# jizongFox/Self-paced-Contrastive-Learning

Measured on AMD Instinct MI355X. Metric: pretrain slices/sec/node (UNet+InfoNCE, 224^2, bs=32/GPU), higher is better.
Workload: dtype bf16; 1 GPU; BASELINE.json configs[1]: self-paced pretrain step, UNet base (max_channel=256) encoder to Conv5 + ProjectionHead(256,256,256) + SelfPacedSupConLoss(soft, partition labels, correct_grad) fwd+bwd + RAdam; slices_per_gpu=32, images_per_gpu_step=64, image=1x224x224, global_batch=32, parallelism=dp1, params=1311056, hipgraph=epocher, capture_steps=3

## Files before the change

include/spcl_hip.h:

```cpp
#ifndef SPCL_HIP_H
#define SPCL_HIP_H
#include <stddef.h>
#include <stdint.h>
#ifdef __cplusplus
extern "C" {
#endif

#define SPCL_F32 0
#define SPCL_BF16 1

#define SPCL_OK 0
#define SPCL_EINVAL (-1)
#define SPCL_ELAUNCH (-2)
#define SPCL_EUNSUPPORTED (-3)

#define SPCL_ABI_VERSION 23
int spcl_abi_version(void);
const char* spcl_last_error(void);

size_t spcl_supcon_workspace_bytes(int n, int d);
int spcl_supcon_forward(const float* z1, const float* z2, const float* labels, const float* mask, int n, int d,
                        float temperature, int sp_mode, float gamma, int correct_grad, float* ws, float* out,
                        void* stream);
int spcl_supcon_backward(const float* labels, const float* mask, int n, int d, float temperature, int sp_mode,
                         float gamma, const float* ws_fwd, float* ws_bwd, const float* out_fwd,
                         const float* grad_out, float* dz1, float* dz2, void* stream);
size_t spcl_supcon_bwd_workspace_bytes(int n, int d);
int spcl_supcon_unit_gradient_block(int n, int d, size_t* offset_floats, int* row_pitch);
int spcl_supcon_forward_heads(int K, const float* z1, const float* z2, size_t z_stride, const float* labels, int n,
                              int d, float temperature, int sp_mode, const float* gammas, int correct_grad, float* ws,
                              size_t ws_stride, float* out, void* stream);
int spcl_supcon_rows_supported(int n, int d);
int spcl_supcon_forward_rows(int K, const float* o1, const float* o2, size_t o_stride, const float* labels, int n, int d,
                             float temperature, int sp_mode, const float* gammas, int correct_grad, float* ws,
                             size_t ws_stride, float* out, void* stream);
int spcl_supcon_backward_heads(int K, const float* labels, int n, int d, float temperature, int sp_mode,
                               const float* gammas, const float* ws_fwd, size_t ws_stride, float* ws_bwd,
                               size_t wsb_stride, const float* out_fwd, const float* grad_out, float* dz1, float* dz2,
                               size_t z_stride, void* stream);
int spcl_supcon_materialize(const float* labels, const float* mask, int n, int d, float temperature, int sp_mode,
                            float gamma, const float* ws_fwd, float* sim_logits, float* sim_exp, float* pos_mask,
                            float* neg_mask, float* sp_mask, void* stream);

size_t spcl_supcon_xpos_workspace_bytes(int n, int d);
int spcl_supcon_xpos_forward(const float* z1, const float* z2, const float* labels, const float* mask, int n, int d,
                             float temperature, float* ws, float* out, void* stream);
int spcl_supcon_xpos_backward(const float* z1, const float* z2, int n, int d, float temperature, const float* ws,
                              const float* grad_out, float* dz1, float* dz2, void* stream);

// ... 172 lines not shown
int spcl_bnrelu_backward_bcast(const void* y, const void* dact_nc, int dtype, int N, int H, int W, int C, int CS,
                               const float* mean, const float* invstd, const float* scale, const float* shift, int training,
                               float* ws, float* dgamma, float* dbeta, void* dy, void* stream);

size_t spcl_bnrelu_image_wgrad_workspace_bytes(int N, int H, int W, int CS);
int spcl_bnrelu_backward_image_wgrad(const void* y, const void* dact, const float* image, int dtype, int N, int H,
                                     int W, int C, int CS, const float* mean, const float* invstd, const float* scale,
                                     const float* shift, int training, float* ws, float* dgamma, float* dbeta,
                                     float* dw, void* stream);

int spcl_conv_dgrad_bnstats_supported(int dtype, int N, int H, int W, int CinK, int CoutS);
int spcl_conv3x3_dgrad_bnstats(const void* dy, int dtype, int N, int H, int W, int CinK, int CoutS, const void* w_packed,
                               void* g, const void* y2, const float* scale2, const float* shift2, const float* mean2,
                               float* rows2, void* stream);

int spcl_image_autocorr_rows(int N, int H, int W);
int spcl_image_autocorr(const float* image, int N, int H, int W, float* out, void* stream);
int spcl_conv_dgrad_bnstats_image_supported(int dtype, int N, int H, int W, int CinK, int CoutS);
int spcl_conv3x3_dgrad_bnstats_image(const void* dy, int dtype, int N, int H, int W, int CinK, int CoutS,
                                     const void* w_packed, void* g, const void* y2, const float* scale2,
                                     const float* shift2, const float* mean2, const float* image, float* rows11,
                                     void* stream);
int spcl_conv16_bwd_fused_supported(int dtype, int N, int H, int W, int CinK, int CoutS);
int spcl_conv16_bwd_fused_splits(int N, int H, int W);
int spcl_conv16_bwd_fused(const void* dy, int dtype, int N, int H, int W, const void* w_packed_dgrad, const void* y2,
                          const float* scale2, const float* shift2, const float* mean2, const float* image,
                          float* rows11, float* partial, float* dw_oihw, int Cin, int Cout, float* wg_rows,
                          const float* acorr, int nacorr, float* acorr16, void* stream);
int spcl_conv16_bwd_fused_image_supported(int dtype, int N, int H, int W, int CinK, int CoutS);
int spcl_conv16_bwd_fused_image(const void* dy, int dtype, int N, int H, int W, const void* w_packed_dgrad,
                                const void* w_packed_image, const float* scale2, const float* shift2, const float* mean2,
                                const float* image, float* rows11, float* partial, float* dw_oihw, int Cin, int Cout,
                                float* wg_rows, const float* acorr, int nacorr, float* acorr16, void* stream);
int spcl_bnrelu_backward_wgrows_image3(const float* wg_rows, int nwg, const float* acorr, int nacorr, const float* w_oihw,
                                       int N, int H, int W, int C, int CS, const float* mean, const float* invstd,
                                       const float* scale, int training, float* ws, float* dgamma, float* dbeta,
                                       float* dw, void* stream);
size_t spcl_bnrelu_image3_workspace_bytes(int CS);
int spcl_bnrelu_backward_rows_image3(const float* rows11, int nrows, const float* acorr, int nacorr, const float* w_oihw,
                                     int N, int H, int W, int C, int CS, const float* mean, const float* invstd,
                                     const float* scale, int training, float* ws, float* dgamma, float* dbeta, float* dw,
                                     void* stream);

int spcl_conv_dgrad_poolstats_supported(int dtype, int N, int H, int W, int CinK, int CoutS, int H2, int W2);
int spcl_conv3x3_dgrad_poolstats(const void* dy, int dtype, int N, int H, int W, int CinK, int CoutS, const void* w_packed,
                                 void* g, const void* y2, int H2, int W2, const float* scale2, const float* shift2,
                                 const float* mean2, float* rows2, void* stream);
int spcl_bnrelu_pool_backward_rows(const void* y, const void* dpool, const float* rows, int nrows, int dtype, int N, int H,
                                   int W, int C, int CS, const float* mean, const float* invstd, const float* scale,
                                   const float* shift, int training, float* ws, float* dgamma, float* dbeta, void* dy,
                                   void* stream);
int spcl_bnrelu_backward_rows(const void* y, const void* dact, const float* image, const float* rows, int nrows, int dtype,
                              int N, int H, int W, int C, int CS, const float* mean, const float* invstd,
                              const float* scale, const float* shift, int training, float* ws, float* dgamma,
                              float* dbeta, void* dy, float* dw, void* stream);


int spcl_conv1x1_forward(const void* x, int dtype, size_t npix, int C, int CS, int K, const float* w, const float* b,
                         float* out, void* stream);
size_t spcl_conv1x1_bwd_workspace_bytes(int C, int K);
int spcl_conv1x1_backward(const void* x, const float* dout, int dtype, size_t npix, int C, int CS, int K, const float* w,
                          void* dx, float* dw, float* db, float* ws, void* stream);
int spcl_conv1x1_forward_bn(const void* y, int dtype, size_t npix, int C, int CS, int K, const float* scale,
                            const float* shift, const float* w, const float* b, float* out, void* stream);
int spcl_conv1x1_bwd_rows(size_t npix);
int spcl_conv1x1_backward_bn(const void* y, const float* dout, int dtype, size_t npix, int C, int CS, int K,
// ... 232 lines not shown
```

self-paced-contrastive-learning_amd/functional.py:

```python
from __future__ import annotations

import ctypes
import math
import os
from ctypes import c_double, c_float, c_int

import torch

from . import native as _n

SP_NONE, SP_HARD, SP_SOFT = 0, 1, 2


def take_grad_sink(param, needed: bool = True):
    if not needed or param is None:
        return None
    sink = getattr(param, "_grad_sink", None)
    if sink is None or not getattr(param, "_grad_sink_armed", False):
        return None
    if sink.shape != param.shape or sink.dtype != torch.float32 or not sink.is_contiguous() or sink.device != param.device:
        return None
    param._grad_sink_armed = False
    return sink

# ... 1357 lines not shown
_CONV16_FUSED = os.environ.get("SPCL_CONV16_FUSED", "1") != "0"
_CONV16_WGROWS = os.environ.get("SPCL_CONV16_WGROWS", "1") != "0"


def _conv16_bwd_fused(dy, wp_t, y2, st2, image, dt_code, N, H, W, cin, cout, cs, sink, acorr=None, wp_image=None):
    dev = dy.device
    if y2 is None and wp_image is None:
        raise RuntimeError("conv16 backward: neither the first convolution's output nor its packed weights")
    nsplit = _n.call("spcl_conv16_bwd_fused_splits", N, H, W)
    if acorr is not None:
        rows = torch.empty(11 * cs * nsplit, dtype=torch.float32, device=dev)
        rows.wg, rows.acorr16 = nsplit, torch.empty(16, 64, dtype=torch.float32, device=dev)
    else:
        nt = _n.call("spcl_conv_stat_rows", dt_code, N, H, W, cs, cs)
        rows = torch.empty(nt * 11 * cs, dtype=torch.float32, device=dev)
        rows.ntiles, rows.wg = nt, 0
    ws = torch.empty(nsplit * 9 * 256, dtype=torch.float32, device=dev)
    dw = _grad_buffer(sink, (cout, cin, 3, 3), dev)

    def launch():
        _n.call("spcl_conv16_bwd_fused" if y2 is not None else "spcl_conv16_bwd_fused_image", _n.ptr(dy), dt_code, N, H, W,
                _n.ptr(wp_t), _n.ptr(y2 if y2 is not None else wp_image), _n.ptr(st2[2]),
                _n.ptr(st2[3]), _n.ptr(st2[0]), _n.ptr(image), _n.ptr(rows) if not rows.wg else None, _n.ptr(ws), _n.ptr(dw),
                cin, cout, _n.ptr(rows) if rows.wg else None, _n.ptr(acorr), 0 if acorr is None else acorr.shape[0],
                _n.ptr(rows.acorr16) if rows.wg else None, _n.stream())

    queue = sink_queue(sink)
    if queue is not None and _TAILS:
        if queue.capture_tail(sink, (ws, dy, y2, image, rows, wp_image), launch):
            return None, rows
        return dw, rows
    launch()
    return dw, rows


def _bnrelu_bwd_rows_image3(rows, acorr, w, N, H, W, C, cs, st, training, sinks):
    dev = rows.device
    ws = torch.empty(_n.call("spcl_bnrelu_image3_workspace_bytes", cs) // 4, dtype=torch.float32, device=dev)
    dw = _grad_buffer(sinks[0], (C, 1, 3, 3), dev)
    dgamma, dbeta = _grad_buffer(sinks[1], (C,), dev), _grad_buffer(sinks[2], (C,), dev)
    wc = w.detach().contiguous().float()
    if getattr(rows, "wg", 0):
        _n.call("spcl_bnrelu_backward_wgrows_image3", _n.ptr(rows), rows.wg, _n.ptr(rows.acorr16), 16, _n.ptr(wc), N, H, W, C,
                cs, _n.ptr(st[0]), _n.ptr(st[1]), _n.ptr(st[2]), int(training), _n.ptr(ws), _n.ptr(dgamma), _n.ptr(dbeta),
                _n.ptr(dw), _n.stream())
        return dw, dgamma, dbeta
    _n.call("spcl_bnrelu_backward_rows_image3", _n.ptr(rows), rows.ntiles, _n.ptr(acorr), acorr.shape[0], _n.ptr(wc), N, H,
            W, C, cs, _n.ptr(st[0]), _n.ptr(st[1]), _n.ptr(st[2]), int(training), _n.ptr(ws), _n.ptr(dgamma), _n.ptr(dbeta),
            _n.ptr(dw), _n.stream())
    return dw, dgamma, dbeta


def _bnrelu_pool_bwd_rows(y, dpool, rows, dt_code, dtype, N, H, W, C, cs, st, training, sinks):
    dev = y.device
    ws = torch.empty(_n.call("spcl_bnrelu_bwd_workspace_bytes", N, H, W, cs) // 4, dtype=torch.float32, device=dev)
    dgamma = _grad_buffer(sinks[0], (C,), dev)
    dbeta = _grad_buffer(sinks[1], (C,), dev)
    dy = torch.empty(N, H, W, cs, dtype=dtype, device=dev)
    _n.call("spcl_bnrelu_pool_backward_rows", _n.ptr(y), _n.ptr(dpool), _n.ptr(rows), rows.ntiles, dt_code, N, H, W, C, cs,
            _n.ptr(st[0]), _n.ptr(st[1]), _n.ptr(st[2]), _n.ptr(st[3]), int(training), _n.ptr(ws), _n.ptr(dgamma),
            _n.ptr(dbeta), _n.ptr(dy), _n.stream())
    return dy, dgamma, dbeta


ACC_ROWS = object()

# ... 260 lines not shown
                dyb, dgb, dbb = _bnrelu_bwd_acc(yb, None, dp_s, None, dtc, dtype, N, H, W, cout, cout_s, stb, cfg.training,
                                                sk[4:6], _take_acc(ctx, "acc_bwd_b"))
            else:
                acc = _take_acc(ctx, "acc_bwd_b") if (_ACC_FILL and H % 2 == 0 and W % 2 == 0 and cout_s <= 256) else None
                if acc is not None:
                    dyb, dgb, dbb = _bnrelu_bwd_rows_acc(yb, None, dp_s, lk.rows, dtc, dtype, N, H, W, cout, cout_s, stb,
                                                         cfg.training, sk[4:6], acc)
                else:
                    dyb, dgb, dbb = _bnrelu_pool_bwd_rows(yb, dp_s, lk.rows, dtc, dtype, N, H, W, cout, cout_s, stb,
                                                          cfg.training, sk[4:6])
        else:
            acc = _take_acc(ctx, "acc_bwd_b") if _ACC_FILL else None
            if acc is not None and lk is not None and lk.rows is ACC_ROWS:
                acc = None
            if acc is not None:
                dyb, dgb, dbb = _bnrelu_bwd_fill(yb, da_s, dp_s, dtc, dtype, N, H, W, cout, cout_s, stb, cfg.training, sk[4:6],
                                                 acc, dact_stride=da_stride, d_up=d_up)
            else:
                dyb, dgb, dbb = _bnrelu_bwd(yb, da_s, dp_s, dtc, dtype, N, H, W, cout, cout_s, stb, cfg.training, sk[4:6],
                                            dact_stride=da_stride, d_up=d_up)
        if lk is not None:
            lk.rows, lk.dx_ptr, lk.holder = None, 0, None
        if la is not None:
            la.rows, la.dx_ptr, la.holder = None, 0, None
        wpa_t, wpb_t = ctx.packed_t
        if wpb_t is None:
            wpb_t = _pack(wb, 1, dtc, dtype)
        image3 = ctx.acorr is not None
        one_pass = (image3 and (_CONV16_FUSED or ya is None) and ctx.needs_input_grad[4] and cout == cout_s
                    and _n.call("spcl_conv16_bwd_fused_supported", dtc, N, H, W, cout_s, cout_s))
        if ya is None and not one_pass:
            raise RuntimeError("image block backward: the first convolution's output was not stored and the one-pass kernel "
                               "that forms it again is not available")
        if one_pass:
            dwb, rows16 = _conv16_bwd_fused(dyb, wpb_t, ya, sta, xs, dtc, N, H, W, cout, cout, cout_s, sk[3],
                                            acorr=ctx.acorr if _CONV16_WGROWS else None, wp_image=ctx.wpa_fwd)
        else:
            dwb = _wgrad(ya, dyb, dtc, N, H, W, cout, cout_s, cout_s, cout, cout_s, 1, sta[2], sta[3], sk[3]) \
                if ctx.needs_input_grad[4] else None
        if one_pass:
            fused = (None, rows16)
        elif image3:
            fused = _dgrad_bnstats_image(dyb, wpb_t, ya, sta, xs, dtc, dtype, N, H, W, cout_s)
        else:
            acc = _take_acc(ctx, "acc_bwd_a")
            if acc is not None:
                fused = (_dgrad_bnstats_acc(dyb, wpb_t, ya, sta, dtc, dtype, N, H, W, cout_s, cout_s, acc), (ACC_ROWS, acc))
            else:
                fused = _dgrad_bnstats(dyb, wpb_t, ya, sta, dtc, dtype, N, H, W, cout_s, cout_s) \
                    if dtype == torch.bfloat16 else None
        if fused is not None:
            daa, rows = fused
        else:
            daa, _ = _conv(dyb, dtc, dtype, N, H, W, cout_s, cout_s, cout_s, wpb_t, 0, None, None, False)
        image_fused = ctx.needs_input_grad[1] and not ctx.needs_input_grad[0] and _image_wgrad_fusable(cfg, cin, cout_s)
        if image3:
            dya = None
            dwa, dga, dba = _bnrelu_bwd_rows_image3(rows, ctx.acorr, wa, N, H, W, cout, cout_s, sta, cfg.training, sk[0:3])
        elif image_fused:
            dya = None
            if fused is not None:
                dwa, dga, dba = _bnrelu_bwd_rows(ya, daa, xs, rows, dtc, dtype, N, H, W, cout, cout_s, sta, cfg.training,
                                                 sk[0:3])
            else:
                dwa, dga, dba = _bnrelu_bwd_image_wgrad(ya, daa, xs, dtc, N, H, W, cout, cout_s, sta, cfg.training,
                                                        sk[0:3])
        else:
            if fused is not None and isinstance(rows, tuple) and rows[0] is ACC_ROWS:
                dya, dga, dba = _bnrelu_bwd_acc(ya, daa, None, None, dtc, dtype, N, H, W, cout, cout_s, sta, cfg.training,
                                                sk[1:3], rows[1])
            elif fused is not None:
                acc = _take_acc(ctx, "acc_rows_a")
                if acc is not None:
                    dya, dga, dba = _bnrelu_bwd_rows_acc(ya, daa, None, rows, dtc, dtype, N, H, W, cout, cout_s, sta,
# ... 1460 lines not shown
```

self-paced-contrastive-learning_amd/native.py:

```python
from __future__ import annotations

import ctypes
import os
from ctypes import c_char_p, c_double, c_float, c_int, c_long, c_size_t, c_void_p

import torch

HERE = os.path.dirname(os.path.abspath(__file__))
LIB_PATH = os.path.join(HERE, "lib", "libspcl_hip.so")
SPCL_F32, SPCL_BF16 = 0, 1

_lib = None

_P = c_void_p
_SIGNATURES = {
    "spcl_abi_version": (c_int, []),
    "spcl_last_error": (c_char_p, []),
    "spcl_supcon_workspace_bytes": (c_size_t, [c_int, c_int]),
    "spcl_supcon_forward": (c_int, [_P, _P, _P, _P, c_int, c_int, c_float, c_int, c_float, c_int, _P, _P, _P]),
    "spcl_supcon_backward": (c_int, [_P, _P, c_int, c_int, c_float, c_int, c_float, _P, _P, _P, _P, _P, _P, _P]),
    "spcl_supcon_bwd_workspace_bytes": (c_size_t, [c_int, c_int]),
    "spcl_supcon_unit_gradient_block": (c_int, [c_int, c_int, _P, _P]),
    "spcl_supcon_materialize": (c_int, [_P, _P, c_int, c_int, c_float, c_int, c_float, _P, _P, _P, _P, _P, _P, _P]),
    "spcl_supcon_xpos_workspace_bytes": (c_size_t, [c_int, c_int]),
# ... 75 lines not shown
    "spcl_bnrelu_backward_up2": (c_int, [_P, _P, _P, c_int, c_int, c_int, c_int, c_int, c_int, _P, _P, _P, _P, c_int, _P, _P, _P, _P,
                                         _P]),
    "spcl_bnrelu_backward_bcast": (c_int, [_P, _P, c_int, c_int, c_int, c_int, c_int, c_int, _P, _P, _P, _P, c_int, _P, _P,
                                           _P, _P, _P]),
    "spcl_bnrelu_image_wgrad_workspace_bytes": (c_size_t, [c_int, c_int, c_int, c_int]),
    "spcl_bnrelu_backward_image_wgrad": (c_int, [_P, _P, _P, c_int, c_int, c_int, c_int, c_int, c_int, _P, _P, _P, _P,
                                                 c_int, _P, _P, _P, _P, _P]),
    "spcl_accumulate_scalars": (c_int, [c_int, _P, _P, _P, _P]),
    "spcl_stage_bytes": (c_int, [_P, _P, c_size_t, _P]),
    "spcl_conv_dgrad_bnstats_supported": (c_int, [c_int, c_int, c_int, c_int, c_int, c_int]),
    "spcl_conv3x3_dgrad_bnstats": (c_int, [_P, c_int, c_int, c_int, c_int, c_int, c_int, _P, _P, _P, _P, _P, _P, _P, _P]),
    "spcl_conv_dgrad_poolstats_supported": (c_int, [c_int, c_int, c_int, c_int, c_int, c_int, c_int, c_int]),
    "spcl_conv3x3_dgrad_poolstats": (c_int, [_P, c_int, c_int, c_int, c_int, c_int, c_int, _P, _P, _P, c_int, c_int, _P, _P,
                                             _P, _P, _P]),
    "spcl_bnrelu_pool_backward_rows": (c_int, [_P, _P, _P, c_int, c_int, c_int, c_int, c_int, c_int, c_int, _P, _P, _P, _P,
                                               c_int, _P, _P, _P, _P, _P]),
    "spcl_bnrelu_backward_rows": (c_int, [_P, _P, _P, _P, c_int, c_int, c_int, c_int, c_int, c_int, c_int, _P, _P, _P, _P,
                                          c_int, _P, _P, _P, _P, _P, _P]),
    "spcl_image_autocorr_rows": (c_int, [c_int, c_int, c_int]),
    "spcl_image_autocorr": (c_int, [_P, c_int, c_int, c_int, _P, _P]),
    "spcl_conv_dgrad_bnstats_image_supported": (c_int, [c_int, c_int, c_int, c_int, c_int, c_int]),
    "spcl_conv3x3_forward_image_acorr_rows": (c_int, [c_int, c_int, c_int, c_int, c_int, c_int]),
    "spcl_conv3x3_forward_image_acorr": (c_int, [_P, c_int, c_int, c_int, c_int, c_int, c_int, _P, _P, _P, _P, _P]),
    "spcl_block1_recompute_supported": (c_int, [c_int, c_int, c_int, c_int, c_int, c_int]),
    "spcl_block1_kernels_take": (c_int, [c_int, c_int, c_int, c_int, c_int, c_int]),
    "spcl_conv3x3_forward_from_image": (c_int, [_P, _P, c_int, c_int, c_int, c_int, c_int, _P, _P, _P, _P, _P, _P, _P]),
    "spcl_conv16_bwd_fused_image_supported": (c_int, [c_int, c_int, c_int, c_int, c_int, c_int]),
    "spcl_conv16_bwd_fused_image": (c_int, [_P, c_int, c_int, c_int, c_int, _P, _P, _P, _P, _P, _P, _P, _P, _P, c_int, c_int,
                                            _P, _P, c_int, _P, _P]),
    "spcl_conv16_bwd_fused_supported": (c_int, [c_int, c_int, c_int, c_int, c_int, c_int]),
    "spcl_conv16_bwd_fused_splits": (c_int, [c_int, c_int, c_int]),
    "spcl_conv16_bwd_fused": (c_int, [_P, c_int, c_int, c_int, c_int, _P, _P, _P, _P, _P, _P, _P, _P, _P, c_int, c_int,
                                      _P, _P, c_int, _P, _P]),
    "spcl_bnrelu_backward_wgrows_image3": (c_int, [_P, c_int, _P, c_int, _P, c_int, c_int, c_int, c_int, c_int, _P, _P, _P,
                                                   c_int, _P, _P, _P, _P, _P]),
    "spcl_conv3x3_dgrad_bnstats_image": (c_int, [_P, c_int, c_int, c_int, c_int, c_int, c_int, _P, _P, _P, _P, _P, _P, _P,
                                                 _P, _P]),
    "spcl_bnrelu_image3_workspace_bytes": (c_size_t, [c_int]),
    "spcl_bnrelu_backward_rows_image3": (c_int, [_P, c_int, _P, c_int, _P, c_int, c_int, c_int, c_int, c_int, _P, _P, _P,
                                                 c_int, _P, _P, _P, _P, _P]),
    "spcl_conv1x1_forward": (c_int, [_P, c_int, c_size_t, c_int, c_int, c_int, _P, _P, _P, _P]),
    "spcl_conv1x1_bwd_workspace_bytes": (c_size_t, [c_int, c_int]),
    "spcl_conv1x1_backward": (c_int, [_P, _P, c_int, c_size_t, c_int, c_int, c_int, _P, _P, _P, _P, _P, _P]),
    "spcl_conv1x1_forward_bn": (c_int, [_P, c_int, c_size_t, c_int, c_int, c_int, _P, _P, _P, _P, _P, _P]),
    "spcl_conv1x1_bwd_rows": (c_int, [c_size_t]),
    "spcl_conv1x1_backward_bn": (c_int, [_P, _P, c_int, c_size_t, c_int, c_int, c_int, _P, _P, _P, _P, _P, _P, _P, _P, _P, _P]),
    "spcl_softmax_forward": (c_int, [_P, c_size_t, c_int, _P, _P]),
    "spcl_softmax_backward": (c_int, [_P, _P, c_size_t, c_int, _P, _P]),
    "spcl_kl_workspace_bytes": (c_size_t, []),
    "spcl_kl_div_forward": (c_int, [_P, _P, c_size_t, c_int, c_float, _P, _P, _P]),
    "spcl_kl_div_backward": (c_int, [_P, _P, c_size_t, c_int, c_float, _P, _P, _P]),
    "spcl_sup_loss_forward": (c_int, [_P, _P, c_int, c_int, c_int, c_float, _P, _P, _P, _P, _P, _P]),
    "spcl_one_hot": (c_int, [_P, c_size_t, c_int, _P, _P]),
    "spcl_argmax_classes": (c_int, [_P, c_size_t, c_int, _P, _P]),
    "spcl_dice_counts": (c_int, [_P, _P, c_int, c_int, c_int, _P, _P, _P]),
    "spcl_surface_workspace_bytes": (c_size_t, [c_int, c_int, c_int, c_int]),
    "spcl_surface_distances": (c_int, [_P, _P, c_int, c_int, c_int, c_int, _P, c_int, c_double, c_double, c_double, _P, _P, _P,
                                       _P, _P, c_size_t, _P]),
    "spcl_surface_3d_workspace_bytes": (c_size_t, [c_int, c_int, c_int, c_int, c_int]),
    "spcl_surface_distances_3d": (c_int, [_P, _P, c_int, c_int, c_int, c_int, c_int, _P, c_int, c_double, c_double, c_double,
                                          c_double, _P, _P, _P, _P, _P, c_size_t, _P]),
    "spcl_upsample2x_forward": (c_int, [_P, _P, c_int, c_int, c_int, c_int, c_int, _P]),
    "spcl_upsample2x_backward": (c_int, [_P, _P, c_int, c_int, c_int, c_int, c_int, _P]),
    "spcl_concat2_channels": (c_int, [_P, _P, _P, c_int, c_size_t, c_int, c_int, _P]),
    "spcl_split2_channels": (c_int, [_P, _P, _P, c_int, c_size_t, c_int, c_int, _P]),
    "spcl_augment_views": (c_int, [_P, c_int, c_int, c_int, _P, c_int, _P, c_int, c_int, _P]),
# ... 101 lines not shown
class WgradItem(ctypes.Structure):
    _fields_ = [("x", c_void_p), ("dy", c_void_p), ("in_scale", c_void_p), ("in_shift", c_void_p),
                ("dw_oihw", c_void_p), ("N", c_int), ("H", c_int), ("W", c_int), ("Cin", c_int), ("CinS", c_int),
                ("Cout", c_int), ("CoutS", c_int), ("in_mode", c_int), ("x2", c_void_p), ("x_up2", c_int)]


class PackItem(ctypes.Structure):
    _fields_ = [("w_oihw", c_void_p), ("fwd", c_void_p), ("dgrad", c_void_p), ("Cin", c_int), ("Cout", c_int),
                ("H", c_int), ("W", c_int)]


BN_EVAL_MAX = 32


class BnEvalItem(ctypes.Structure):
    _fields_ = [("gamma", c_void_p), ("beta", c_void_p), ("running_mean", c_void_p), ("running_var", c_void_p),
                ("st", c_void_p), ("C", c_int), ("CS", c_int), ("eps", c_float)]


class BnAcc(ctypes.Structure):
    _fields_ = [("acc", c_void_p), ("gamma", c_void_p), ("beta", c_void_p), ("running_mean", c_void_p),
                ("running_var", c_void_p), ("num_batches_tracked", c_void_p), ("st", c_void_p), ("momentum", c_float),
                ("eps", c_float), ("count", c_float), ("C", c_int), ("CS", c_int)]


PACK_MULTI_MAX = 24


class WgradTail(ctypes.Structure):
    _fields_ = [("partial", c_void_p), ("dw", c_void_p), ("kind", c_int), ("nsplit", c_int), ("nblk_ci", c_int),
                ("nblk_co", c_int), ("CIB", c_int), ("COB", c_int), ("Cin", c_int), ("Cout", c_int)]


ABI_VERSION = 23
WGRAD_BATCH_MAX = 16
WGRAD_TAILS_MAX = 16
_NO_STATUS = ("spcl_abi_version", "spcl_block1_recompute_supported", "spcl_block1_kernels_take", "spcl_conv16_bwd_fused_image_supported", "spcl_conv3x3_forward_image_acorr_rows", "spcl_image_autocorr_rows", "spcl_conv_dgrad_bnstats_image_supported", "spcl_conv16_bwd_fused_supported", "spcl_conv16_bwd_fused_splits", "spcl_conv_num_tiles", "spcl_conv_stat_rows", "spcl_conv_set_gemm", "spcl_conv_set_f32_split", "spcl_conv_get_f32_split", "spcl_supcon_unit_gradient_block", "spcl_conv_cat_supported", "spcl_conv_up2_supported", "spcl_conv_split_supported", "spcl_conv_split_bnstats_supported", "spcl_conv1x1_bwd_rows", "spcl_profile_count", "spcl_conv_dgrad_bnstats_supported", "spcl_conv_dgrad_poolstats_supported",
              "spcl_conv_wgrad_batched_supported", "spcl_conv_bn_acc_supported", "spcl_conv_dgrad_bnstats_acc_supported",
              "spcl_conv_dgrad_poolstats_acc_supported", "spcl_supcon_rows_supported", "spcl_bnrelu_gap_supported",
              "spcl_conv_dgrad_poolmax_supported", "spcl_conv_dgrad_poolmax_acc_supported")


class NativeLibraryError(RuntimeError):
    pass


def lib():
    global _lib
    if _lib is None:
        if not os.path.exists(LIB_PATH):
            raise NativeLibraryError(
                f"{LIB_PATH} is missing: build it with `python self-paced-contrastive-learning_amd/build.py` "
                "(there is no CPU / eager fallback for the hot path)")
        L = ctypes.CDLL(LIB_PATH)
        L.spcl_abi_version.restype, L.spcl_abi_version.argtypes = c_int, []
        have = L.spcl_abi_version()
        if have != ABI_VERSION:
            raise NativeLibraryError(
                f"{LIB_PATH} has C-ABI version {have}, this binding was written for {ABI_VERSION} (include/spcl_hip.h "
                "SPCL_ABI_VERSION): a stale build -- rebuild with `python self-paced-contrastive-learning_amd/build.py`")
        for name, (res, args) in _SIGNATURES.items():
            fn = getattr(L, name, None)
            if fn is None:
                continue
            fn.restype, fn.argtypes = res, args
        _lib = L
    return _lib


def call(name: str, *args):
    L = lib()
    fn = getattr(L, name, None)
    if fn is None:
# ... 35 lines not shown
```

Baseline: 32590 slices/s.

## Fuse dgrad, BN-ReLU stats and wgrad for 32-channel conv backward

Adds a single HIP kernel for the 32->32 channel 3x3 conv backward in encoder blocks. One pass computes the data gradient, writes it as bf16, accumulates BN backward statistics, and recomputes the BN-ReLU input into LDS so the weight gradient can be accumulated with MFMA in the same kernel. The halo load for the next image is software-pipelined behind the current one. This replaces the separate wgrad and dgrad+bnstats kernels, removing a second read of dy and y2. The cost is higher register and LDS pressure plus a per-workgroup partial buffer that still needs a reduction.

```diff
diff --git a/include/spcl_hip.h b/include/spcl_hip.h
--- a/include/spcl_hip.h
+++ b/include/spcl_hip.h
@@ -14,7 +14,7 @@
 #define SPCL_ELAUNCH (-2)
 #define SPCL_EUNSUPPORTED (-3)
 
-#define SPCL_ABI_VERSION 23
+#define SPCL_ABI_VERSION 24
 int spcl_abi_version(void);
 const char* spcl_last_error(void);
 
@@ -253,6 +253,11 @@
                                 const void* w_packed_image, const float* scale2, const float* shift2, const float* mean2,
                                 const float* image, float* rows11, float* partial, float* dw_oihw, int Cin, int Cout,
                                 float* wg_rows, const float* acorr, int nacorr, float* acorr16, void* stream);
+int spcl_conv32_bwd_fused_supported(int dtype, int N, int H, int W, int CinK, int CoutS);
+int spcl_conv32_bwd_fused_splits(int N, int H, int W);
+int spcl_conv32_bwd_fused(const void* dy, int dtype, int N, int H, int W, const void* w_packed_dgrad, const void* y2,
+                          const float* scale2, const float* shift2, const float* mean2, void* g, float* rows,
+                          float* partial, float* dw_oihw, int Cin, int Cout, void* stream);
 int spcl_bnrelu_backward_wgrows_image3(const float* wg_rows, int nwg, const float* acorr, int nacorr, const float* w_oihw,
                                        int N, int H, int W, int C, int CS, const float* mean, const float* invstd,
                                        const float* scale, int training, float* ws, float* dgamma, float* dbeta,
diff --git a/self-paced-contrastive-learning_amd/csrc/conv32_bwd.hip b/self-paced-contrastive-learning_amd/csrc/conv32_bwd.hip
--- /dev/null
+++ b/self-paced-contrastive-learning_amd/csrc/conv32_bwd.hip
@@ -0,0 +1,303 @@
+#include "conv_common.hpp"
+
+namespace spcl {
+
+struct Bwd32Args {
+  const unsigned char* dy;
+  const u32x4* wp;
+  const unsigned char* y2;
+  const float* scale2;
+  const float* shift2;
+  const float* mean2;
+  unsigned char* g;
+  float* rows;
+  float* partial;
+  int N, H, W, tilesX, tilesY, ipw, xcd_remap;
+};
+
+constexpr int C32_TH = 14, C32_TW = 14, C32_HW = 16, C32_RP = 18, C32_PS = 96, C32_PIX = 64;
+constexpr int C32_DY = 0, C32_DY_BYTES = (C32_TH + 2) * C32_RP * C32_PS;
+constexpr int C32_XT = C32_DY_BYTES, C32_XT_ROW = 16 * C32_PS, C32_XT_BYTES = C32_TH * C32_XT_ROW;
+constexpr int C32_LDS = C32_XT + C32_XT_BYTES;
+#ifndef SPCL_CONV32_WG_PER_CU
+#define SPCL_CONV32_WG_PER_CU 2
+#endif
+
+__device__ __forceinline__ bf16x8 c32_tr_frag(unsigned addr) {
+  const s16x4 lo = __builtin_amdgcn_ds_read_tr16_b64_v4i16((s16x4 __attribute__((address_space(3)))*)(uintptr_t)addr);
+  const s16x4 hi =
+      __builtin_amdgcn_ds_read_tr16_b64_v4i16((s16x4 __attribute__((address_space(3)))*)(uintptr_t)(addr + 8 * C32_PS));
+  return __builtin_shufflevector(lo, hi, 0, 1, 2, 3, 4, 5, 6, 7);
+}
+
+__global__ __launch_bounds__(256) __attribute__((amdgpu_waves_per_eu(2))) void conv32_bwd_kernel(Bwd32Args a) {
+  constexpr int TH = C32_TH, TW = C32_TW, RP = C32_RP, PS = C32_PS, PIX = C32_PIX;
+  constexpr int NW = 4, MW = TH / 2, UPW = 5, NUNIT = 18;
+  extern __shared__ __attribute__((aligned(16))) unsigned char lds[];
+  const unsigned lds_base = (unsigned)(uintptr_t)(unsigned char __attribute__((address_space(3)))*)lds;
+  const int t0 = threadIdx.x;
+  const int wave = __builtin_amdgcn_readfirstlane(t0 >> 6);
+  const int nt = wave & 1, rw = wave >> 1;
+
+  int tx = blockIdx.x, ty = blockIdx.y;
+  {
+    const int T = a.tilesX * a.tilesY;
+    if (a.xcd_remap && (T & 7) == 0) {
+      const int L = ty * a.tilesX + tx;
+      const int L2 = (L & 7) * (T >> 3) + (L >> 3);
+      ty = L2 / a.tilesX;
+      tx = L2 - ty * a.tilesX;
+    }
+  }
+  const int y0 = ty * TH, x0 = tx * TW;
+  const bool interior = y0 > 0 && x0 > 0 && y0 + TH < a.H && x0 + TW < a.W;
+
+  if (t0 < 128) *(u32x4*)(lds + C32_DY + ((t0 >> 3) * RP + C32_HW + ((t0 >> 2) & 1)) * PS + (t0 & 3) * 16) = (u32x4){0u, 0u, 0u, 0u};
+  f32x4 wacc[UPW][2];
+#pragma unroll
+  for (int j = 0; j < UPW; ++j) wacc[j][0] = wacc[j][1] = (f32x4){0.f, 0.f, 0.f, 0.f};
+
+  u32x4 v[4];
+  uint2 ypre[MW];
+  auto rsrc = [](const void* p) { return __builtin_amdgcn_make_buffer_rsrc((void*)p, 0, 0x7fffffff, 0x00020000); };
+  constexpr int OOB = (int)0x80000000u;
+  auto issue_halo = [&](const int n, const bool live) {
+    int t = t0;
+    asm volatile("" : "+v"(t));
+    const int ch = t & 3, q0 = t >> 2, hy0 = q0 >> 4, hx0 = q0 & 15;
+    const int voff = (hy0 * a.W + hx0) * PIX + ch * 16;
+    const __amdgpu_buffer_rsrc_t rs = rsrc(a.dy + (((long)n * a.H + (y0 - 1)) * a.W + (x0 - 1)) * PIX);
+#pragma unroll
+    for (int k = 0; k < 4; ++k) {
+      bool inb = live;
+      if (!interior) {
+        const int gy = y0 - 1 + hy0 + 4 * k, gx = x0 - 1 + hx0;
+        inb = live && gy >= 0 && gy < a.H && gx >= 0 && gx < a.W;
+      }
+      v[k] = __builtin_bit_cast(u32x4, __builtin_amdgcn_raw_buffer_load_b128(rs, inb ? voff : OOB, 4 * k * a.W * PIX, 0));
+    }
+  };
+  auto issue_y2 = [&](const int n) {
+    int t = t0;
+    asm volatile("" : "+v"(t));
+    const int r16 = t & 15, g = (t & 63) >> 4;
+    const int voff = min(r16, TW - 1) * PIX + nt * 32 + g * 8;
+    const __amdgpu_buffer_rsrc_t rs = rsrc(a.y2 + (((size_t)n * a.H + y0 + MW * rw) * a.W + x0) * PIX);
+#pragma unroll
+    for (int j = 0; j < MW; ++j)
+      ypre[j] = __builtin_bit_cast(uint2, __builtin_amdgcn_raw_buffer_load_b64(rs, voff, j * a.W * PIX, 0));
+  };
+
+  const int n_first = blockIdx.z * a.ipw;
+  if (n_first < a.N) {
+    issue_halo(n_first, true);
+    issue_y2(n_first);
+  }
+  u32x4 wall[9];
+  f32x4 sc2, sh2, mu2;
+  {
+    const int lane = t0 & 63, g = lane >> 4;
+    const __amdgpu_buffer_rsrc_t rs_wp = rsrc(a.wp), rs_sc = rsrc(a.scale2), rs_sh = rsrc(a.shift2), rs_mu = rsrc(a.mean2);
+#pragma unroll
+    for (int s = 0; s < 9; ++s)
+      wall[s] = __builtin_bit_cast(u32x4, __builtin_amdgcn_raw_buffer_load_b128(rs_wp, lane * 16, (s * 2 + nt) * 1024, 0));
+    sc2 = __builtin_bit_cast(f32x4, __builtin_amdgcn_raw_buffer_load_b128(rs_sc, g * 16, nt * 64, 0));
+    sh2 = __builtin_bit_cast(f32x4, __builtin_amdgcn_raw_buffer_load_b128(rs_sh, g * 16, nt * 64, 0));
+    mu2 = __builtin_bit_cast(f32x4, __builtin_amdgcn_raw_buffer_load_b128(rs_mu, g * 16, nt * 64, 0));
+    if ((t0 & 15) >= TW) {
+      sc2 = (f32x4){0.f, 0.f, 0.f, 0.f};
+      sh2 = (f32x4){-1.f, -1.f, -1.f, -1.f};
+    }
+#pragma unroll
+    for (int s = 0; s < 9; ++s) asm volatile("" : "+v"(wall[s]));
+    asm volatile("" : "+v"(sc2), "+v"(sh2), "+v"(mu2));
+  }
+
+  auto second_half = [&]() {
+    int t = t0;
+    asm volatile("" : "+v"(t));
+    const int r16 = t & 15, g = (t & 63) >> 4;
+    __syncthreads();
+    const unsigned tr_col = (unsigned)((4 * (g & 1) + (r16 >> 2)) * PS + (r16 & 3) * 8);
+    const unsigned ax = lds_base + C32_XT + (g >> 1) * C32_XT_ROW + tr_col;
+    unsigned ad[UPW];
+#pragma unroll
+    for (int j = 0; j < UPW; ++j) {
+      const int u = min(wave + NW * j, NUNIT - 1), tap = u >> 1, cot = u & 1, ky = tap / 3, kx = tap - 3 * ky;
+      ad[j] = lds_base + C32_DY + ((g >> 1) + 2 - ky) * RP * PS + tr_col + (2 - kx) * PS + cot * 32;
+    }
+#pragma unroll
+    for (int ks = 0; ks < TH / 2; ++ks) {
+      const bf16x8 af0 = c32_tr_frag(ax + ks * 2 * C32_XT_ROW), af1 = c32_tr_frag(ax + 32 + ks * 2 * C32_XT_ROW);
+#pragma unroll
+      for (int j = 0; j < UPW; ++j) {
+        const bf16x8 bf = c32_tr_frag(ad[j] + ks * 2 * RP * PS);
+        wacc[j][0] = __builtin_amdgcn_mfma_f32_16x16x32_bf16(af0, bf, wacc[j][0], 0, 0, 0);
+        wacc[j][1] = __builtin_amdgcn_mfma_f32_16x16x32_bf16(af1, bf, wacc[j][1], 0, 0, 0);
+      }
+      __builtin_amdgcn_sched_barrier(0);
+    }
+    __syncthreads();
+  };
+
+  int n = n_first;
+  if (n_first < a.N)
+#pragma unroll 1
+  for (int it = 0;; ++it, ++n) {
+    int t = t0;
+    asm volatile("" : "+v"(t));
+    const int r16 = t & 15, g = (t & 63) >> 4;
+    {
+      const int ch = t & 3, q0 = t >> 2, hy0 = q0 >> 4, hx0 = q0 & 15;
+      unsigned char* const lp = lds + C32_DY + (hy0 * RP + hx0) * PS + ch * 16;
+#pragma unroll
+      for (int k = 0; k < 4; ++k) *(u32x4*)(lp + (4 * k * RP) * PS) = v[k];
+    }
+    const bool more = it + 1 < a.ipw && n + 1 < a.N;
+    issue_halo(n + 1, more);
+    __syncthreads();
+
+    const unsigned lb = (unsigned)(C32_DY + (MW * rw * RP + r16) * PS + g * 16);
+    const unsigned xaddr = (unsigned)(C32_XT + MW * rw * C32_XT_ROW + r16 * PS + nt * 32 + g * 8);
+    unsigned char* const gp = a.g + (((size_t)n * a.H + y0 + MW * rw) * a.W + x0 + min(r16, TW - 1)) * PIX + nt * 32 + g * 8;
+    const int grow = a.W * PIX;
+    uint2 gpk[MW];
+    auto store_g = [&]() {
+      if (r16 < TW) {
+#pragma unroll
+        for (int j = 0; j < MW; ++j) *(uint2*)(gp + (size_t)j * grow) = gpk[j];
+      }
+    };
+    f32x4 ssum = {0.f, 0.f, 0.f, 0.f}, ssq = {0.f, 0.f, 0.f, 0.f};
+#pragma unroll
+    for (int j = 0; j < MW; ++j) {
+      f32x4 acc = {0.f, 0.f, 0.f, 0.f};
+#pragma unroll
+      for (int s = 0; s < 9; ++s) {
+        const int ky = s / 3, kx = s - 3 * ky;
+        const u32x4 xf = *(const u32x4*)(lds + lb + ((j + ky) * RP + kx) * PS);
+        acc = mfma_chunk<bf16_t>(wall[s], xf, acc);
+      }
+      const uint2 yr = ypre[j];
+      const float yv[4] = {__uint_as_float(yr.x << 16), __uint_as_float(yr.x & 0xffff0000u),
+                           __uint_as_float(yr.y << 16), __uint_as_float(yr.y & 0xffff0000u)};
+      const f32x2 glo = {acc[0], acc[1]}, ghi = {acc[2], acc[3]};
+      const uint32_t g0 = __builtin_bit_cast(uint32_t, __builtin_convertvector(glo, bf16x2v));
+      const uint32_t g1 = __builtin_bit_cast(uint32_t, __builtin_convertvector(ghi, bf16x2v));
+      gpk[j] = (uint2){g0, g1};
+      asm volatile("" : "+v"(gpk[j].x), "+v"(gpk[j].y));
+      const float gv[4] = {__uint_as_float(g0 << 16), __uint_as_float(g0 & 0xffff0000u),
+                           __uint_as_float(g1 << 16), __uint_as_float(g1 & 0xffff0000u)};
+      float xv[4];
+#pragma unroll
+      for (int r = 0; r < 4; ++r) {
+        const float z = fmaf(sc2[r], yv[r], sh2[r]);
+        xv[r] = z;
+        const float dz = z > 0.f ? gv[r] : 0.f;
+        ssum[r] += dz;
+        ssq[r] = fmaf(dz, yv[r] - mu2[r], ssq[r]);
+      }
+      const f32x2 lo = {xv[0], xv[1]}, hi = {xv[2], xv[3]};
+      uint2 w;
+      w.x = relu_bf16x2(__builtin_bit_cast(uint32_t, __builtin_convertvector(lo, bf16x2v)));
+      w.y = relu_bf16x2(__builtin_bit_cast(uint32_t, __builtin_convertvector(hi, bf16x2v)));
+      *(uint2*)(lds + xaddr + j * C32_XT_ROW) = w;
+      __builtin_amdgcn_sched_barrier(0);
+    }
+    {
+      f32x4 o;
+#pragma unroll
+      for (int r = 0; r < 4; ++r) {
+        const float s1 = row16_sum(ssum[r]), s2 = row16_sum(ssq[r]);
+        o[r] = r16 == 0 ? s1 : s2;
+      }
+      const size_t set = ((size_t)n * 2 * a.tilesY + 2 * ty + rw) * a.tilesX + tx;
+      if (r16 < 2) *(f32x4*)(a.rows + (set * 2 + r16) * 32 + nt * 16 + 4 * g) = o;
+    }
+    if (!more) {
+      store_g();
+      break;
+    }
+    issue_y2(n + 1);
+    store_g();
+    second_half();
+  }
+  if (n_first < a.N) second_half();
+
+  const size_t wg = (size_t)(blockIdx.z * gridDim.y + blockIdx.y) * gridDim.x + blockIdx.x;
+  float* out = a.partial + wg * (9 * 32 * 32);
+#pragma unroll
+  for (int j = 0; j < UPW; ++j) {
+    const int u = wave + NW * j;
+    if (u < NUNIT) {
+      const int tap = u >> 1, cot = u & 1;
+#pragma unroll
+      for (int cit = 0; cit < 2; ++cit)
+#pragma unroll
+        for (int r = 0; r < 4; ++r)
+          out[(tap * 32 + cit * 16 + 4 * ((t0 & 63) >> 4) + r) * 32 + cot * 16 + (t0 & 15)] = wacc[j][cit][r];
+    }
+  }
+}
+
+static int conv32_bwd_ipw(int N, int H, int W) {
+  static const int per_cu = lab_env("SPCL_CONV32_WG_PER_CU", SPCL_CONV32_WG_PER_CU);
+  const int resident = 256 * (per_cu < 1 ? 1 : (per_cu > 2 ? 2 : per_cu));
+  const long tiles = (long)(H / C32_TH) * (W / C32_TW);
+  static const int env_ipw = lab_env("SPCL_CONV32_IPW", 0);
+  int ipw = env_ipw > 0 ? env_ipw : (int)((tiles * N + resident - 1) / resident);
+  if (ipw < 1) ipw = 1;
+  if (ipw > N) ipw = N;
+  return ipw;
+}
+
+}
+
+using namespace spcl;
+
+extern "C" int spcl_conv32_bwd_fused_supported(int dtype, int N, int H, int W, int CinK, int CoutS) {
+  static const bool off = lab_flag("SPCL_NO_CONV32_FUSED");
+  return (!off && dtype == SPCL_BF16 && CinK == 32 && CoutS == 32 && N > 0 && H >= C32_TH && W >= C32_TW && H % C32_TH == 0 &&
+          W % C32_TW == 0 && (double)H * W * 64.0 < 2147483648.0)
+             ? 1 : 0;
+}
+
+extern "C" int spcl_conv32_bwd_fused_splits(int N, int H, int W) {
+  if (N <= 0 || H < C32_TH || W < C32_TW || H % C32_TH != 0 || W % C32_TW != 0) return 0;
+  return (H / C32_TH) * (W / C32_TW) * cdiv(N, conv32_bwd_ipw(N, H, W));
+}
+
+extern "C" int spcl_conv32_bwd_fused(const void* dy, int dtype, int N, int H, int W, const void* w_packed_dgrad, const void* y2,
+                                     const float* scale2, const float* shift2, const float* mean2, void* g, float* rows,
+                                     float* partial, float* dw_oihw, int Cin, int Cout, void* stream) {
+  SPCL_CHECK_ARG(dy && w_packed_dgrad && y2 && scale2 && shift2 && mean2 && g && rows && partial && dw_oihw,
+                 "conv32_bwd_fused: null pointer");
+  SPCL_CHECK_ARG(Cin > 0 && Cin <= 32 && Cout > 0 && Cout <= 32, "conv32_bwd_fused: channel counts");
+  SPCL_CHECK_ARG((uintptr_t)dy % 16 == 0 && (uintptr_t)y2 % 16 == 0 && (uintptr_t)g % 16 == 0,
+                 "conv32_bwd_fused: tensors must be 16-byte aligned");
+  if (!spcl_conv32_bwd_fused_supported(dtype, N, H, W, 32, 32)) {
+    set_error("conv32_bwd_fused: unsupported configuration (bf16, 32 -> 32 channels, H and W multiples of 14)");
+    return SPCL_EUNSUPPORTED;
+  }
+  hipStream_t st = (hipStream_t)stream;
+  spcl_wgrad_tail* tail = take_tail_capture();
+  Bwd32Args a;
+  a.dy = (const unsigned char*)dy; a.wp = (const u32x4*)w_packed_dgrad; a.y2 = (const unsigned char*)y2;
+  a.scale2 = scale2; a.shift2 = shift2; a.mean2 = mean2; a.g = (unsigned char*)g; a.rows = rows; a.partial = partial;
+  a.N = N; a.H = H; a.W = W; a.tilesX = W / C32_TW; a.tilesY = H / C32_TH;
+  a.ipw = conv32_bwd_ipw(N, H, W);
+  static const int env_remap = lab_env("SPCL_CONV_XCD_REMAP", 1);
+  a.xcd_remap = env_remap;
+  const int nz = cdiv(N, a.ipw), nsplit = a.tilesX * a.tilesY * nz;
+  const double px = (double)N * H * W;
+  prof_cost(px * 64.0 * 3.0 + (double)nsplit * 9 * 1024 * 4.0, 2.0 * 2.0 * px * 9.0 * 32 * 32);
+  SPCL_LAUNCH(conv32_bwd_kernel, dim3(a.tilesX, a.tilesY, nz), dim3(256), C32_LDS, st, a);
+  if (tail != nullptr) {
+    tail->partial = partial; tail->dw = dw_oihw; tail->kind = 0; tail->nsplit = nsplit; tail->nblk_ci = 1;
+    tail->nblk_co = 1; tail->CIB = 32; tail->COB = 32; tail->Cin = Cin; tail->Cout = Cout;
+  } else {
+    launch_wgrad_reduce(partial, nsplit, 1, 1, 32, 32, Cin, Cout, dw_oihw, st);
+  }
+  SPCL_LAUNCH_CHECK("conv32_bwd_fused");
+  return SPCL_OK;
+}
diff --git a/self-paced-contrastive-learning_amd/functional.py b/self-paced-contrastive-learning_amd/functional.py
--- a/self-paced-contrastive-learning_amd/functional.py
+++ b/self-paced-contrastive-learning_amd/functional.py
@@ -1413,6 +1413,32 @@
         return dw, rows
     launch()
     return dw, rows
+
+
+_CONV32_FUSED = os.environ.get("SPCL_CONV32_FUSED", "1") != "0"
+
+
+def _conv32_bwd_fused(dy, wp_t, y2, st2, dt_code, dtype, N, H, W, cin, cout, cs, sink):
+    dev = dy.device
+    nsplit = _n.call("spcl_conv32_bwd_fused_splits", N, H, W)
+    g = torch.empty(N, H, W, cs, dtype=dtype, device=dev)
+    nrows = 2 * N * (H // 14) * (W // 14)
+    rows = torch.empty(nrows * 2 * cs, dtype=torch.float32, device=dev)
+    rows.ntiles = nrows
+    ws = torch.empty(nsplit * 9 * cs * cs, dtype=torch.float32, device=dev)
+    dw = _grad_buffer(sink, (cout, cin, 3, 3), dev)
+
+    def launch():
+        _n.call("spcl_conv32_bwd_fused", _n.ptr(dy), dt_code, N, H, W, _n.ptr(wp_t), _n.ptr(y2), _n.ptr(st2[2]),
+                _n.ptr(st2[3]), _n.ptr(st2[0]), _n.ptr(g), _n.ptr(rows), _n.ptr(ws), _n.ptr(dw), cin, cout, _n.stream())
+
+    queue = sink_queue(sink)
+    if queue is not None and _TAILS:
+        if queue.capture_tail(sink, (ws, dy, y2, g, rows), launch):
+            return None, g, rows
+        return dw, g, rows
+    launch()
+    return dw, g, rows
 
 
 def _bnrelu_bwd_rows_image3(rows, acorr, w, N, H, W, C, cs, st, training, sinks):
@@ -1739,14 +1765,21 @@
         if ya is None and not one_pass:
             raise RuntimeError("image block backward: the first convolution's output was not stored and the one-pass kernel "
                                "that forms it again is not available")
+        one_pass32 = (not image3 and _CONV32_FUSED and dtype == torch.bfloat16 and ya is not None
+                      and ctx.needs_input_grad[4] and cout == cout_s and getattr(ctx, "acc_bwd_a", None) is None
+                      and _n.call("spcl_conv32_bwd_fused_supported", dtc, N, H, W, cout_s, cout_s))
         if one_pass:
             dwb, rows16 = _conv16_bwd_fused(dyb, wpb_t, ya, sta, xs, dtc, N, H, W, cout, cout, cout_s, sk[3],
                                             acorr=ctx.acorr if _CONV16_WGROWS else None, wp_image=ctx.wpa_fwd)
+        elif one_pass32:
+            dwb, g32, rows32 = _conv32_bwd_fused(dyb, wpb_t, ya, sta, dtc, dtype, N, H, W, cout, cout, cout_s, sk[3])
         else:
             dwb = _wgrad(ya, dyb, dtc, N, H, W, cout, cout_s, cout_s, cout, cout_s, 1, sta[2], sta[3], sk[3]) \
                 if ctx.needs_input_grad[4] else None
         if one_pass:
             fused = (None, rows16)
+        elif one_pass32:
+            fused = (g32, rows32)
         elif image3:
             fused = _dgrad_bnstats_image(dyb, wpb_t, ya, sta, xs, dtc, dtype, N, H, W, cout_s)
         else:
diff --git a/self-paced-contrastive-learning_amd/native.py b/self-paced-contrastive-learning_amd/native.py
--- a/self-paced-contrastive-learning_amd/native.py
+++ b/self-paced-contrastive-learning_amd/native.py
@@ -131,6 +131,9 @@
     "spcl_conv16_bwd_fused_splits": (c_int, [c_int, c_int, c_int]),
     "spcl_conv16_bwd_fused": (c_int, [_P, c_int, c_int, c_int, c_int, _P, _P, _P, _P, _P, _P, _P, _P, _P, c_int, c_int,
                                       _P, _P, c_int, _P, _P]),
+    "spcl_conv32_bwd_fused_supported": (c_int, [c_int, c_int, c_int, c_int, c_int, c_int]),
+    "spcl_conv32_bwd_fused_splits": (c_int, [c_int, c_int, c_int]),
+    "spcl_conv32_bwd_fused": (c_int, [_P, c_int, c_int, c_int, c_int, _P, _P, _P, _P, _P, _P, _P, _P, _P, c_int, c_int, _P]),
     "spcl_bnrelu_backward_wgrows_image3": (c_int, [_P, c_int, _P, c_int, _P, c_int, c_int, c_int, c_int, c_int, _P, _P, _P,
                                                    c_int, _P, _P, _P, _P, _P]),
     "spcl_conv3x3_dgrad_bnstats_image": (c_int, [_P, c_int, c_int, c_int, c_int, c_int, c_int, _P, _P, _P, _P, _P, _P, _P,
@@ -298,13 +301,14 @@
                 ("nblk_co", c_int), ("CIB", c_int), ("COB", c_int), ("Cin", c_int), ("Cout", c_int)]
 
 
-ABI_VERSION = 23
+ABI_VERSION = 24
 WGRAD_BATCH_MAX = 16
 WGRAD_TAILS_MAX = 16
 _NO_STATUS = ("spcl_abi_version", "spcl_block1_recompute_supported", "spcl_block1_kernels_take", "spcl_conv16_bwd_fused_image_supported", "spcl_conv3x3_forward_image_acorr_rows", "spcl_image_autocorr_rows", "spcl_conv_dgrad_bnstats_image_supported", "spcl_conv16_bwd_fused_supported", "spcl_conv16_bwd_fused_splits", "spcl_conv_num_tiles", "spcl_conv_stat_rows", "spcl_conv_set_gemm", "spcl_conv_set_f32_split", "spcl_conv_get_f32_split", "spcl_supcon_unit_gradient_block", "spcl_conv_cat_supported", "spcl_conv_up2_supported", "spcl_conv_split_supported", "spcl_conv_split_bnstats_supported", "spcl_conv1x1_bwd_rows", "spcl_profile_count", "spcl_conv_dgrad_bnstats_supported", "spcl_conv_dgrad_poolstats_supported",
               "spcl_conv_wgrad_batched_supported", "spcl_conv_bn_acc_supported", "spcl_conv_dgrad_bnstats_acc_supported",
               "spcl_conv_dgrad_poolstats_acc_supported", "spcl_supcon_rows_supported", "spcl_bnrelu_gap_supported",
-              "spcl_conv_dgrad_poolmax_supported", "spcl_conv_dgrad_poolmax_acc_supported")
+              "spcl_conv_dgrad_poolmax_supported", "spcl_conv_dgrad_poolmax_acc_supported",
+              "spcl_conv32_bwd_fused_supported", "spcl_conv32_bwd_fused_splits")
 
 
 class NativeLibraryError(RuntimeError):
```

Result: no change. 32800 slices/s, median of 6 (+0.7%).
